# LMCache/LMCache

Measured on NVIDIA H100. Metric: kv_encode_decode_raw_GBps, higher is better.
Workload: dtype f32->u8 (bf16 KV)

## Files before the change

### lmcache_b200/csrc/codec.cu

```cuda
#include <cuda_bf16.h>
#include <cuda_fp16.h>
#include <cuda_runtime.h>
#include <stdint.h>
#include <stdlib.h>
#include <string.h>

#include <algorithm>
#include <vector>

#include "ac_core.cuh"
#include "common.cuh"

namespace b200kv {

constexpr int CT = 128;
constexpr int SPW = 6;
constexpr int SYMW = 43;
constexpr int PAIRW = 33;
constexpr int TEMPW_FUSED = 40;
constexpr int TEMPW_SPLIT = 132;
constexpr int TEMPW_FUSED_RANS = 48;
constexpr int CODER_AC = 0, CODER_RANS = 1;
constexpr int CODER_RANS_COMPACT = 2;
constexpr int kHdrRowWords = 8;
// ... 6 lines not shown
    int32_t L, H, D, C, dtype;
    int32_t n_chunks, chunk_tokens, last_chunk_tokens, tpp;
    int32_t tiles_full, tempw;
    int32_t stage_bytes;
    int32_t coder;
    int32_t compact;
    int32_t ppl;
    uint8_t* out;
    int64_t out_stride;
    uint64_t* sizes_out;
    uint32_t* temp;
    uint32_t* rstate;
    uint32_t* tile_tot;
    unsigned long long* totals;
    unsigned int* err;
    int32_t lb, nlay;
    uint8_t* arena;
    int64_t arena_bytes;
    unsigned long long* chunk_base;
    unsigned long long* cursor;
    unsigned int* fail_from;
    unsigned long long* ptotal;
    int64_t* seg;
    int32_t layers_left;
};
static_assert(sizeof(EncParams) < kMaxParamBytes, "EncParams must stay under 4 KB of kernel parameters");

__device__ __forceinline__ int launch_plane(const EncParams& P, int local) {
    return local + (local < P.nlay ? P.lb : P.L - P.nlay + P.lb);
}
// ... 47 lines not shown
    if (nb > 16) m |= (uint32_t)*reinterpret_cast<const uint16_t*>(p + 2) << 16;
    if (nb <= 8) m &= 0xffu;
    return nb >= 32 ? m : m & ((1u << nb) - 1u);
}

__device__ __forceinline__ int chunk_tokens_of(const EncParams& P, int j) {
    return j == P.n_chunks - 1 ? P.last_chunk_tokens : P.chunk_tokens;
}

template <bool PAGED>
__device__ __forceinline__ int64_t tok_row(const int64_t* slot_map, int64_t tok) {
    if constexpr (PAGED) return __ldg(slot_map + tok);
    else return tok;
}

template <bool VEC, bool PAGED>
__global__ void __launch_bounds__(256) absmax_kernel(EncParams P, int64_t total_tokens) {
    const int64_t warp = (blockIdx.x * (int64_t)blockDim.x + threadIdx.x) >> 5;
    const int lane = threadIdx.x & 31;
    const int64_t nrows = (int64_t)P.ppl * P.nlay * total_tokens;
    if (warp >= nrows) return;
    const int nl = launch_plane(P, (int)(warp / total_tokens));
    const int64_t T = warp % total_tokens;
    const uint16_t* row = P.pt.p[nl] + tok_row<PAGED>(P.slot_map, P.tok_begin + T) * P.sT;
    uint32_t m = 0;
    if (VEC) {
        const int vec_per_head = P.D >> 3;
        const int nvec = P.H * vec_per_head;
        for (int v = lane; v < nvec; v += 32) {
            const int h = v / vec_per_head, dv = v - h * vec_per_head;
            const uint4 q = __ldg(reinterpret_cast<const uint4*>(row + (int64_t)h * P.sH + dv * 8));
            const uint32_t w[4] = {q.x, q.y, q.z, q.w};
#pragma unroll
            for (int k = 0; k < 4; ++k) {
                const uint32_t a = w[k] & 0x7fff7fffu;
                m = max(m, max(a & 0xffffu, a >> 16));
            }
        }
    } else {
        for (int c = lane; c < P.C; c += 32) {
            const int h = c / P.D, d = c - h * P.D;
            m = max(m, (uint32_t)(__ldg(row + (int64_t)h * P.sH + d) & 0x7fffu));
        }
    }
    m = __reduce_max_sync(0xffffffffu, m);
    if (lane == 0) {
        const int j = (int)(T / P.chunk_tokens);
        const int tj = chunk_tokens_of(P, j);
        const Layout lo = layout_of(P, tj);
        uint16_t* maxes = reinterpret_cast<uint16_t*>(P.out + (int64_t)j * P.out_stride + lo.off_maxes);
        maxes[(int64_t)nl * tj + (T - (int64_t)j * P.chunk_tokens)] = (uint16_t)m;
    }
}

__device__ __forceinline__ uint32_t block_excl_scan(uint32_t v, uint32_t* s_warp, uint32_t* total) {
    const int lane = threadIdx.x & 31, wid = threadIdx.x >> 5;
    uint32_t inc = v;
#pragma unroll
    for (int o = 1; o < 32; o <<= 1) {
        uint32_t n = __shfl_up_sync(0xffffffffu, inc, o);
// ... 82 lines not shown
        for (int k = BT - 1; k >= 0; --k)
            if (tk + k < gt) f(q[k]);
    };
    load(xa, nbatch - 1);
    for (int b = nbatch - 1; b >= 0; b -= 2) {
        if (b >= 1) load(xb, b - 1);
        use(xa, b);
        if (b >= 1) {
            if (b >= 2) load(xa, b - 2);
            use(xb, b - 1);
        }
    }
}


template <bool FUSED, int DT, bool PAGED, int CODER>
__global__ void __launch_bounds__(CT, FUSED ? 7 : 4) encode_kernel(EncParams P) {
    extern __shared__ __align__(128) uint32_t smem[];
    constexpr int ROWS_W = FUSED ? CT * SYMW : 0;
    constexpr int TAB_W = FUSED ? (CT * kLp * 2 + 3) / 4 : CT * PAIRW;
    uint32_t* rows = smem;
    uint32_t* tab = smem + ROWS_W;
    float* fac = reinterpret_cast<float*>(smem + ((ROWS_W + TAB_W + 3) & ~3));
    __shared__ uint32_t s_warp[CT / 32];

    const int tid = threadIdx.x;
    TileId id;
    if (!decode_tile(P, blockIdx.x, &id)) return;
    const int NL = P.ppl * P.L;
    const int j = id.j, nl = id.nl, ct = id.ct, t = id.t, gt = id.gt;
    const int c = ct * CT + tid;
    const bool active = c < P.C;
    const int ncols = min(CT, P.C - ct * CT);

    uint8_t* cont = P.out + (int64_t)j * P.out_stride;
    const Layout lo = layout_of(P, t);
    const uint16_t* maxes = reinterpret_cast<const uint16_t*>(cont + lo.off_maxes) + (int64_t)nl * t + id.tok0;
    const float maxq = P.pt.maxq[nl];
    const int64_t s1 = P.sT;
    for (int i = tid; i < gt; i += CT)
        fac[i] = FUSED ? quant_factor_safe(maxq, half_to_float(maxes[i], DT)) : quant_factor(maxq, half_to_float(maxes[i], DT));
    if (FUSED) for (int i = gt + tid; i < kGroup + 8; i += CT) fac[i] = 0.0f;

    const int h = active ? c / P.D : 0;
    const int64_t tokabs = P.tok_begin + (int64_t)j * P.chunk_tokens + id.tok0;
    const uint16_t* cbase = P.pt.p[nl] + (int64_t)h * P.sH + (active ? c - h * P.D : 0);
    const uint16_t* src = cbase + (PAGED ? 0 : tokabs * P.sT);
    uint32_t* trow = P.temp + ((int64_t)blockIdx.x * CT + tid) * P.tempw;
    uint32_t cap = (uint32_t)P.tempw;
    asm volatile("" : "+l"(trow), "+r"(cap));
    uint32_t len = 0u, hlen = 0u;

    if (FUSED) {
        uint32_t* myrow = rows + tid * SYMW;
        uint16_t* cdfr = reinterpret_cast<uint16_t*>(tab);
        uint16_t* crow = cdfr + tid * kLp;
        uint16_t* hist = crow;
#pragma unroll
        for (int i = 0; i < kLp; ++i) crow[i] = 0;
        if (!PAGED) {
            const int lines_per_tok = (ncols * 2 + 127) >> 7;
            const uint16_t* tile0 = P.pt.p[nl] + (P.tok_begin + (int64_t)j * P.chunk_tokens + id.tok0) * P.sT +
                                    (int64_t)((ct * CT) / P.D) * P.sH + ((ct * CT) % P.D);
// ... 76 lines not shown
            uint32_t mask = 0u;
#pragma unroll
            for (int i = 0; i < 32; ++i) mask |= (cnt[i] != 0u ? 1u : 0u) << i;
            const uint32_t wany = __reduce_or_sync(__activemask(), mask);
            CdfAccum2 acc;
            acc.init();
#pragma unroll
            for (uint32_t i = 0; i < 32u; ++i) {
                crow[i] = (uint16_t)acc.value(i);
                if ((wany >> i) & 1u) acc.absorb(fac[cnt[i]]);
            }
            crow[32] = (uint16_t)acc.value(32u);
            if (P.compact) {
                uint32_t w0, w1;
                hlen = build_stream_header(cnt, mask, wany, 2 * ((int)maxq + 1), trow, w0, w1);
                reinterpret_cast<uint2*>(P.rstate)[((int64_t)blockIdx.x * CT + tid) * 2] = make_uint2(w0, w1);
            }
        }
        __syncthreads();
        if (!P.compact) {
            uint16_t* dstc = reinterpret_cast<uint16_t*>(cont + lo.off_cdf) + ((int64_t)nl * P.C + ct * CT) * kLp;
            for (int e = tid; e < ncols * kLp; e += CT) dstc[e] = cdfr[e];
        }
        if (active && CODER == CODER_RANS) {
            uint32_t x = kRansLow;
            const uint16_t* const wend = reinterpret_cast<const uint16_t*>(trow) + 2 * P.tempw;
            int32_t nk = 0;
            const char* const cb = reinterpret_cast<const char*>(crow);
            auto code = [&](uint32_t word, int k) {
                const uint32_t o = (k == 0 ? word << 1 : word >> (5 * k - 1)) & 62u;
                const uint32_t c_lo = *reinterpret_cast<const uint16_t*>(cb + o);
                const uint32_t c_hi = *reinterpret_cast<const uint16_t*>(cb + o + 2);
                rans_put(x, nk, wend, c_lo, c_hi - c_lo);
            };
            int w = (gt - 1) / SPW;
            {
                const uint32_t word = myrow[w];
                for (int k = gt - 1 - w * SPW; k >= 0; --k) code(word, k);
            }
            for (--w; w >= 0; --w) {
                const uint32_t word = myrow[w];
#pragma unroll
                for (int k = SPW - 1; k >= 0; --k) code(word, k);
            }
            if (P.compact) reinterpret_cast<uint2*>(P.rstate)[((int64_t)blockIdx.x * CT + tid) * 2 + 1] = make_uint2(x, hlen);
            else P.rstate[(int64_t)blockIdx.x * CT + tid] = x;
            len = hlen + 4u - 2u * (uint32_t)nk;
        } else if (active) {
            EncState2 st;
            st.init();
            int tk = 0;
            for (int w = 0; tk < gt; ++w) {
                const uint32_t word = myrow[w];
                if (tk + SPW <= gt) {
#pragma unroll
                    for (int k = 0; k < SPW; ++k) {
                        const uint32_t sidx = (word >> (5 * k)) & 31u;
                        const uint32_t c_lo = crow[sidx];
                        enc_symbol2(st, c_lo, (uint32_t)crow[sidx + 1u] - c_lo, trow, cap);
                    }
                    tk += SPW;
// ... 19 lines not shown
#pragma unroll
            for (int i = 0; i < kLp; ++i) cv[i] = prow[i] & 0xffffu;
#pragma unroll
            for (int i = 0; i < 32; ++i) {
                const uint32_t hi = (i == 31) ? 0x10000u : cv[i + 1];
                prow[i] = cv[i] | ((hi - cv[i]) << 16);
            }
            if (CODER == CODER_RANS) {
                uint32_t x = kRansLow;
                const uint16_t* const wend = reinterpret_cast<const uint16_t*>(trow) + 2 * TEMPW_SPLIT;
                int32_t nk = 0;
                for_each_symbol_rev<DT, PAGED, 4>(cbase, P.slot_map, tokabs, s1, gt, fac, maxq, [&](uint32_t q) {
                    const uint32_t pr = prow[q];
                    rans_put(x, nk, wend, pr & 0xffffu, pr >> 16);
                });
                P.rstate[(int64_t)blockIdx.x * CT + tid] = x;
                len = 4u - 2u * (uint32_t)nk;
            } else {
                EncState2 st;
                st.init();
                for_each_symbol<DT, PAGED, 4>(cbase, P.slot_map, tokabs, s1, gt, fac, maxq, [&](uint32_t q) {
                    const uint32_t pr = prow[q];
                    enc_symbol2(st, pr & 0xffffu, pr >> 16, trow, cap);
                });
                len = enc_finish2(st, trow, cap);
                if (st.w > cap) atomicOr(&P.err[j], 1u);
            }
        }
    }

    if (active) store_len(cont + lo.off_lengths, ((int64_t)id.g * NL + nl) * P.C + c, len, P.compact != 0);
    uint32_t tile_total;
    (void)block_excl_scan(len, s_warp, &tile_total);
    if (tid == 0) P.tile_tot[(int64_t)j * P.tiles_full + id.tile_in_chunk] = tile_total;
}

template <int DT, bool PAGED>
__global__ void __launch_bounds__(CT) cdf_kernel(EncParams P) {
    extern __shared__ __align__(128) uint32_t smem[];
    uint32_t* cnts = smem;
    float* fac = reinterpret_cast<float*>(cnts + CT * PAIRW);
    const int tid = threadIdx.x;
    const int NL = P.ppl * P.L;
    const uint32_t per_chunk = (uint32_t)NL * P.tpp;
    const uint32_t j = blockIdx.x / per_chunk;
    const uint32_t rem = blockIdx.x - j * per_chunk;
    const int nl = (int)(rem / P.tpp);
    const int ct = (int)(rem - (uint32_t)nl * P.tpp);
    const int t = chunk_tokens_of(P, (int)j);
// ... 855 lines not shown
        }
        cudaEventRecord(g_prof_ev[slot][0], stream);
    }
    ~ProfScope() {
        if (!g_prof_on) return;
        cudaEventRecord(g_prof_ev[slot][1], stream);
        g_prof_have[slot] = true;
    }
};

static int enc_tempw(bool fused, int coder, bool compact = false) {
    if (compact) return TEMPW_FUSED_RANS_HDR;
    return fused ? (coder == CODER_RANS ? TEMPW_FUSED_RANS : TEMPW_FUSED) : TEMPW_SPLIT;
}

static size_t enc_ws_layout(int64_t n_tiles_alloc, int n_chunks, int tempw, int coder, bool compact, size_t* off_tot,
                            size_t* off_totals, size_t* off_err, size_t* off_state, size_t* off_temp) {
    size_t o = 0;
    *off_tot = o;    o += (size_t)n_tiles_alloc * 4;  o = (o + 255) & ~(size_t)255;
    *off_totals = o; o += (size_t)n_chunks * 8;       o = (o + 255) & ~(size_t)255;
    *off_err = o;    o += (size_t)n_chunks * 4;       o = (o + 255) & ~(size_t)255;
    *off_state = o;  o += coder == CODER_RANS ? (size_t)n_tiles_alloc * CT * (compact ? 16 : 4) : 0;  o = (o + 255) & ~(size_t)255;
    *off_temp = o;   o += (size_t)n_tiles_alloc * CT * (size_t)tempw * 4;
    return (o + 255) & ~(size_t)255;
}

struct EnclWs { size_t err, ptotal, cbase, state, tot, totals, rstate, temp, bytes; };
static EnclWs encl_ws_layout(int n_chunks, int64_t call_tiles) {
    EnclWs w;
    size_t o = 0;
    auto take = [&](size_t* off, size_t n) { *off = o; o = (o + n + 255) & ~(size_t)255; };
    take(&w.err, (size_t)n_chunks * 4);
    take(&w.ptotal, (size_t)n_chunks * 8);
    take(&w.cbase, (size_t)n_chunks * 8);
    take(&w.state, 16);
    take(&w.tot, (size_t)call_tiles * 4);
    take(&w.totals, (size_t)n_chunks * 8);
    take(&w.rstate, (size_t)call_tiles * CT * 16);
    take(&w.temp, (size_t)call_tiles * CT * TEMPW_FUSED_RANS_HDR * 4);
    w.bytes = o;
    return w;
}

constexpr uint32_t kEncPlanMagic = 0x4e4c5045u;
struct LayerSet {
    static constexpr int kWords = B200KV_MAX_PLANES / 2 / 64;
    uint64_t w[kWords];
    static LayerSet range(int a, int b) {
        LayerSet s;
        for (int i = 0; i < kWords; ++i) {
            const int lo = std::max(a - 64 * i, 0), hi = std::min(b - 64 * i, 64);
            s.w[i] = lo >= hi ? 0ull : (hi - lo == 64 ? ~0ull : ((1ull << (hi - lo)) - 1ull) << lo);
// ... 19 lines not shown
        return n;
    }
};
static_assert(LayerSet::kWords * 64 == B200KV_MAX_PLANES / 2, "one bit per layer");
struct EncPlan {
    uint32_t magic;
    int32_t max_layers;
    LayerSet done;
    EncParams P;
};
static_assert(sizeof(EncPlan) <= sizeof(b200kv_encode_plan_t), "b200kv_encode_plan_t too small");

constexpr size_t kSmemFused = (size_t)(((CT * SYMW + (CT * kLp * 2 + 3) / 4 + 3) & ~3) + kGroup + 8) * 4;
constexpr int kStageRans = 12 * 1024;

static int launch_absmax(const EncParams& P, const b200kv_kv_desc* kv, int64_t total_tokens, cudaStream_t stream) {
    bool vec = (kv->D % 8 == 0) && (kv->sT % 8 == 0) && (kv->sH % 8 == 0);
    for (int nl = 0; nl < P.ppl * P.L && vec; ++nl) vec = (reinterpret_cast<uintptr_t>(P.pt.p[nl]) & 15) == 0;
    const bool paged = P.slot_map != nullptr;
    const int64_t rows = (int64_t)P.ppl * P.nlay * total_tokens;
    const int64_t blocks = (rows + 7) / 8;
    B2_REQUIRE(blocks < (1ll << 31), "too many rows in one call");
    if (vec && !paged) absmax_kernel<true, false><<<(unsigned)blocks, 256, 0, stream>>>(P, total_tokens);
    else if (vec) absmax_kernel<true, true><<<(unsigned)blocks, 256, 0, stream>>>(P, total_tokens);
    else if (!paged) absmax_kernel<false, false><<<(unsigned)blocks, 256, 0, stream>>>(P, total_tokens);
    else absmax_kernel<false, true><<<(unsigned)blocks, 256, 0, stream>>>(P, total_tokens);
    B2_CHECK_CUDA(cudaGetLastError());
    return 0;
}

static size_t dec_ws_layout(int64_t tiles_max, int n_chunks, int NP, size_t* off_tb, size_t* off_pt) {
    size_t o = ((size_t)n_chunks * sizeof(DecChunk) + 255) & ~(size_t)255;
    *off_tb = o;
    o += (size_t)n_chunks * (size_t)tiles_max * 8;
    o = (o + 255) & ~(size_t)255;
    *off_pt = o;
    if (NP > kInlinePlanes) o = (o + sizeof(PlaneTable) + 255) & ~(size_t)255;
    return o;
}

constexpr uint32_t kPlanMagic = 0x4e4c5044u;
// ... 70 lines not shown
    return 0;
}

int64_t b200kv_encode_workspace_bytes(int32_t L, int32_t H, int32_t D, int32_t chunk_tokens, int32_t n_chunks,
                                      int32_t coder) {
    if (L <= 0 || H <= 0 || D <= 0 || chunk_tokens <= 0 || n_chunks <= 0) return -2;
    const int ppl = (coder & B200KV_KV_LATENT) ? 1 : 2;
    coder &= 0xff;
    const bool compact = coder == CODER_RANS_COMPACT;
    if (compact) coder = CODER_RANS;
    if (coder != CODER_AC && coder != CODER_RANS) return -2;
    if (compact && chunk_tokens > kGroup) return -2;
    if (ppl == 1 && !compact) return -2;
    const int64_t G = (chunk_tokens + kGroup - 1) / kGroup;
    const int64_t n_tiles = (int64_t)n_chunks * G * ppl * L * tiles_per_plane(H * D);
    size_t a, b, c, d, e;
    return (int64_t)enc_ws_layout(n_tiles, n_chunks, enc_tempw(chunk_tokens <= kGroup, coder, compact), coder, compact, &a, &b, &c, &d, &e);
}

int64_t b200kv_decode_workspace_bytes(int32_t L, int32_t H, int32_t D, int32_t chunk_tokens, int32_t n_chunks) {
    if (L <= 0 || H <= 0 || D <= 0 || chunk_tokens <= 0 || n_chunks <= 0) return -2;
    const int64_t G = (chunk_tokens + kGroup - 1) / kGroup;
    const int64_t tiles_max = G * 2 * L * tiles_per_plane(H * D);
    size_t a, b;
    return (int64_t)dec_ws_layout(tiles_max, n_chunks, 2 * L, &a, &b);
}

int b200kv_encode_chunks(const b200kv_kv_desc* kv, int64_t tok_begin, int32_t n_chunks, int32_t chunk_tokens,
                         int32_t last_chunk_tokens, const float* key_bins, const float* value_bins, int32_t coder,
                         void* out, int64_t out_stride, uint64_t* sizes_out, void* workspace, int64_t workspace_bytes,
                         void* stream_) {
    cudaStream_t stream = static_cast<cudaStream_t>(stream_);
// ... 24 lines not shown
    P.out_stride = out_stride;
    P.sizes_out = sizes_out;
    P.lb = 0; P.nlay = P.L;
    P.arena = nullptr; P.arena_bytes = 0; P.chunk_base = nullptr; P.cursor = nullptr; P.fail_from = nullptr;
    P.ptotal = nullptr; P.seg = nullptr; P.layers_left = 0;
    const Layout lo = make_layout(P.L, P.C, chunk_tokens, P.compact, P.ppl);
    B2_REQUIRE(out_stride >= lo.off_payload + 16, "out_stride smaller than the fixed container sections");

    const int64_t G = lo.ngroups;
    const int64_t per_group = (int64_t)P.ppl * P.L * P.tpp;
    const int64_t tiles_full = G * per_group;
    const int64_t n_tiles = (int64_t)n_chunks * tiles_full;
    const bool fused = chunk_tokens <= kGroup;
    P.tiles_full = (int32_t)tiles_full;
    P.tempw = enc_tempw(fused, coder, P.compact != 0);
    size_t off_tot, off_totals, off_err, off_state, off_temp;
    const size_t need = enc_ws_layout(n_tiles, n_chunks, P.tempw, coder, P.compact != 0, &off_tot, &off_totals, &off_err, &off_state,
                                      &off_temp);
    B2_REQUIRE(workspace != nullptr && workspace_bytes >= (int64_t)need, "workspace too small");
    B2_REQUIRE(n_tiles < (1ll << 31) && tiles_full < (1ll << 31), "too many tiles in one call");
    uint8_t* ws = static_cast<uint8_t*>(workspace);
    P.tile_tot = reinterpret_cast<uint32_t*>(ws + off_tot);
    P.totals = reinterpret_cast<unsigned long long*>(ws + off_totals);
    P.err = reinterpret_cast<unsigned int*>(ws + off_err);
    P.temp = reinterpret_cast<uint32_t*>(ws + off_temp);
    P.rstate = reinterpret_cast<uint32_t*>(ws + off_state);
    B2_CHECK_CUDA(cudaMemsetAsync(ws, 0, off_state, stream));

    const int64_t total_tokens = (int64_t)(n_chunks - 1) * chunk_tokens + last_chunk_tokens;
    for (int i = 0; i <= kProfFinalize; ++i) g_prof_have[i] = false;
    {
        ProfScope prof(kProfAbsmax, stream);
        if (int rc = launch_absmax(P, kv, total_tokens, stream)) return rc;
    }
    const size_t smem_fused = kSmemFused;
    const size_t smem_split = (size_t)(((CT * PAIRW + 3) & ~3) + kGroup + 4) * 4;
    const size_t smem_cdf = (size_t)(CT * PAIRW + kGroup) * 4;
#define B2_LAUNCH_ENC1(FUSED, DT, PAGED, CODER, SMEM)                                                      \
    do {                                                                                                   \
        B2_CHECK_CUDA(cudaFuncSetAttribute(encode_kernel<FUSED, DT, PAGED, CODER>,                         \
                                           cudaFuncAttributeMaxDynamicSharedMemorySize, (int)(SMEM)));     \
        encode_kernel<FUSED, DT, PAGED, CODER><<<(unsigned)n_tiles, CT, (SMEM), stream>>>(P);              \
    } while (0)
#define B2_LAUNCH_ENC(FUSED, DT, PAGED, SMEM)                                                              \
    do {                                                                                                   \
        if (coder == CODER_RANS) B2_LAUNCH_ENC1(FUSED, DT, PAGED, CODER_RANS, SMEM);                       \
        else B2_LAUNCH_ENC1(FUSED, DT, PAGED, CODER_AC, SMEM);                                             \
    } while (0)
#define B2_LAUNCH_ENC2(FUSED, SMEM)                                                                        \
    do {                                                                                                   \
        if (P.dtype == B200KV_DT_BF16) { if (paged) B2_LAUNCH_ENC(FUSED, 0, true, SMEM); else B2_LAUNCH_ENC(FUSED, 0, false, SMEM); } \
        else { if (paged) B2_LAUNCH_ENC(FUSED, 1, true, SMEM); else B2_LAUNCH_ENC(FUSED, 1, false, SMEM); } \
    } while (0)
    if (fused) {
        ProfScope prof(kProfEncode, stream);
        B2_LAUNCH_ENC2(true, smem_fused);
    } else {
        const unsigned cdf_blocks = (unsigned)((int64_t)n_chunks * per_group);
        {
            ProfScope prof(kProfCdf, stream);
            if (P.dtype == B200KV_DT_BF16) {
                if (paged) cdf_kernel<0, true><<<cdf_blocks, CT, smem_cdf, stream>>>(P);
                else cdf_kernel<0, false><<<cdf_blocks, CT, smem_cdf, stream>>>(P);
            } else {
                if (paged) cdf_kernel<1, true><<<cdf_blocks, CT, smem_cdf, stream>>>(P);
                else cdf_kernel<1, false><<<cdf_blocks, CT, smem_cdf, stream>>>(P);
            }
        }
        B2_CHECK_CUDA(cudaGetLastError());
        ProfScope prof(kProfEncode, stream);
        B2_LAUNCH_ENC2(false, smem_split);
// ... 8 lines not shown
        if (coder == CODER_RANS && !hint_mid) P.stage_bytes = 12 * 1024;
        B2_CHECK_CUDA(cudaFuncSetAttribute(compact_kernel, cudaFuncAttributeMaxDynamicSharedMemorySize, P.stage_bytes));
        enc_scan_kernel<<<(unsigned)n_chunks, 1024, 0, stream>>>(P);
        compact_kernel<<<(unsigned)n_tiles, CT, (size_t)P.stage_bytes, stream>>>(P);
        finalize_kernel<<<(n_chunks + 127) / 128, 128, 0, stream>>>(P);
    }
    B2_CHECK_CUDA(cudaGetLastError());
    return 0;
}

int64_t b200kv_encode_layers_workspace_bytes(int32_t L, int32_t H, int32_t D, int32_t chunk_tokens, int32_t n_chunks,
                                             int32_t max_layers) {
    if (L <= 0 || H <= 0 || D <= 0 || chunk_tokens <= 0 || chunk_tokens > kGroup || n_chunks <= 0 || max_layers <= 0 ||
        max_layers > L)
        return -2;
    return (int64_t)encl_ws_layout(n_chunks, (int64_t)n_chunks * 2 * max_layers * tiles_per_plane(H * D)).bytes;
}

int b200kv_encode_layers_plan(const b200kv_kv_desc* kv, int64_t tok_begin, int32_t n_chunks, int32_t chunk_tokens,
                              int32_t last_chunk_tokens, const float* key_bins, const float* value_bins, int32_t coder,
                              void* arena, int64_t arena_bytes, void* fixed_out, int64_t fixed_stride, int64_t* seg_sizes_out,
                              uint64_t* sizes_out, int32_t max_layers, void* workspace, int64_t workspace_bytes,
                              b200kv_encode_plan_t* plan_out, void* stream_) {
    cudaStream_t stream = static_cast<cudaStream_t>(stream_);
    B2_REQUIRE(plan_out != nullptr, "plan is NULL");
    EncPlan* plan = reinterpret_cast<EncPlan*>(plan_out);
    plan->magic = 0u;
    EncParams& P = plan->P;
    B2_REQUIRE(key_bins && value_bins, "bins are NULL");
    B2_REQUIRE((coder & 0xff) == CODER_RANS_COMPACT,
               "the layer-wise encode writes compact containers only (B200KV_CODER_RANS_COMPACT)");
// ... 14 lines not shown
    P.tpp = tiles_per_plane(P.C);
    P.coder = CODER_RANS;
    P.compact = 1;
    P.tempw = TEMPW_FUSED_RANS_HDR;
    P.stage_bytes = kStageRans;
    const Layout lo = make_layout(P.L, P.C, chunk_tokens, 1, P.ppl);
    B2_REQUIRE(fixed_stride >= lo.off_payload, "fixed_stride smaller than the fixed container sections");
    P.out = static_cast<uint8_t*>(fixed_out);
    P.out_stride = fixed_stride;
    P.sizes_out = sizes_out;
    P.arena = static_cast<uint8_t*>(arena);
    P.arena_bytes = arena_bytes;
    P.seg = seg_sizes_out;
    const int64_t call_tiles = (int64_t)n_chunks * P.ppl * max_layers * P.tpp;
    B2_REQUIRE(call_tiles < (1ll << 31), "too many tiles in one call");
    const EnclWs w = encl_ws_layout(n_chunks, call_tiles);
    B2_REQUIRE(workspace != nullptr && workspace_bytes >= (int64_t)w.bytes, "workspace too small");
    uint8_t* ws = static_cast<uint8_t*>(workspace);
    P.err = reinterpret_cast<unsigned int*>(ws + w.err);
    P.ptotal = reinterpret_cast<unsigned long long*>(ws + w.ptotal);
    P.chunk_base = reinterpret_cast<unsigned long long*>(ws + w.cbase);
    P.cursor = reinterpret_cast<unsigned long long*>(ws + w.state);
    P.fail_from = reinterpret_cast<unsigned int*>(ws + w.state + 8);
    P.tile_tot = reinterpret_cast<uint32_t*>(ws + w.tot);
    P.totals = reinterpret_cast<unsigned long long*>(ws + w.totals);
    P.rstate = reinterpret_cast<uint32_t*>(ws + w.rstate);
    P.temp = reinterpret_cast<uint32_t*>(ws + w.temp);
    B2_CHECK_CUDA(cudaMemsetAsync(ws, 0, w.tot, stream));
    B2_CHECK_CUDA(cudaMemsetAsync(fixed_out, 0, (size_t)fixed_stride * n_chunks, stream));
    encl_init_kernel<<<1, 1, 0, stream>>>(P);
    B2_CHECK_CUDA(cudaGetLastError());
    B2_CHECK_CUDA(cudaFuncSetAttribute(compact_kernel, cudaFuncAttributeMaxDynamicSharedMemorySize, P.stage_bytes));
    plan->max_layers = max_layers;
    plan->done = LayerSet::range(0, 0);
    plan->magic = kEncPlanMagic;
    return 0;
}

int b200kv_encode_layers(b200kv_encode_plan_t* plan_in, int32_t layer_begin, int32_t layer_end, void* stream_) {
    cudaStream_t stream = static_cast<cudaStream_t>(stream_);
    B2_REQUIRE(plan_in != nullptr, "plan is NULL");
    EncPlan* plan = reinterpret_cast<EncPlan*>(plan_in);
    B2_REQUIRE(plan->magic == kEncPlanMagic, "not a plan made by b200kv_encode_layers_plan");
    EncParams P = plan->P;
    B2_REQUIRE(layer_begin >= 0 && layer_begin < layer_end && layer_end <= P.L, "layer range out of range");
    B2_REQUIRE(layer_end - layer_begin <= plan->max_layers, "more layers than the plan's workspace holds");
    const LayerSet bits = LayerSet::range(layer_begin, layer_end);
    B2_REQUIRE(!plan->done.intersects(bits), "a layer of the range was encoded before");
    P.lb = layer_begin;
    P.nlay = layer_end - layer_begin;
    P.layers_left = P.L - plan->done.count() - bits.count();
    P.tiles_full = P.ppl * P.nlay * P.tpp;
    const int64_t n_tiles = (int64_t)P.n_chunks * P.tiles_full;
    const int64_t total_tokens = (int64_t)(P.n_chunks - 1) * P.chunk_tokens + P.last_chunk_tokens;
    b200kv_kv_desc kv{};
    kv.D = P.D; kv.sT = P.sT; kv.sH = P.sH;
    if (int rc = launch_absmax(P, &kv, total_tokens, stream)) return rc;
#define B2_LAUNCH_ENCL(DT, PAGED)                                                                                      \
    do {                                                                                                               \
        B2_CHECK_CUDA(cudaFuncSetAttribute(encode_kernel<true, DT, PAGED, CODER_RANS>,                                 \
                                           cudaFuncAttributeMaxDynamicSharedMemorySize, (int)kSmemFused));             \
        encode_kernel<true, DT, PAGED, CODER_RANS><<<(unsigned)n_tiles, CT, kSmemFused, stream>>>(P);                  \
    } while (0)
    if (P.dtype == B200KV_DT_BF16) { if (P.slot_map) B2_LAUNCH_ENCL(0, true); else B2_LAUNCH_ENCL(0, false); }
    else { if (P.slot_map) B2_LAUNCH_ENCL(1, true); else B2_LAUNCH_ENCL(1, false); }
#undef B2_LAUNCH_ENCL
    B2_CHECK_CUDA(cudaGetLastError());
    enc_scan_kernel<<<(unsigned)P.n_chunks, 1024, 0, stream>>>(P);
    place_kernel<<<1, 1024, 0, stream>>>(P);
    compact_kernel<<<(unsigned)n_tiles, CT, (size_t)P.stage_bytes, stream>>>(P);
    B2_CHECK_CUDA(cudaGetLastError());
    plan->done.add(bits);
    return 0;
}

int b200kv_encode_layers_finish(const b200kv_encode_plan_t* plan_in, void* stream_) {
    cudaStream_t stream = static_cast<cudaStream_t>(stream_);
    B2_REQUIRE(plan_in != nullptr, "plan is NULL");
    const EncPlan* plan = reinterpret_cast<const EncPlan*>(plan_in);
    B2_REQUIRE(plan->magic == kEncPlanMagic, "not a plan made by b200kv_encode_layers_plan");
    EncParams P = plan->P;
    B2_REQUIRE(plan->done == LayerSet::range(0, P.L), "a layer was never encoded");
// ... 251 lines not shown
```

Measured before the change: 424.9.

## Fuse absmax into persistent encode kernel with ticket scheduler and ready flags

Replaces the separate absmax launch in the fused encode path with a persistent encode kernel. Its blocks pull work tickets that interleave absmax row-groups and encode tiles, with a lead of a few units so absmax runs ahead. Encode tiles spin on per-unit release/acquire ready counters before reading maxes. This removes a kernel boundary and lets the absmax reads overlap with encoding. It adds atomic ticket contention, spin-waits and a deadlock risk if scheduling assumptions fail. The absmax row loop is also batched four loads deep.

```diff
diff --git a/fused_absmax_bench.py b/fused_absmax_bench.py
--- /dev/null
+++ b/fused_absmax_bench.py
@@ -0,0 +1,109 @@
+#!/usr/bin/env python
+import argparse
+import ctypes
+import json
+import os
+import subprocess
+import sys
+
+ROOT = os.path.dirname(os.path.abspath(__file__))
+sys.path.insert(0, ROOT)
+
+MODEL = "lmsys/longchat-7b-16k"
+L, D = 32, 128
+
+
+def card():
+    try:
+        q = subprocess.run(["nvidia-smi", "--query-gpu=name,power.limit,clocks.max.sm", "--format=csv,noheader"],
+                           capture_output=True, text=True, timeout=30).stdout.strip().splitlines()
+        return q[0] if q else None
+    except (OSError, subprocess.SubprocessError):
+        return None
+
+
+def main():
+    ap = argparse.ArgumentParser()
+    ap.add_argument("--tokens", type=int, default=8192)
+    ap.add_argument("--chunk", type=int, default=256)
+    ap.add_argument("--heads", type=int, default=32)
+    ap.add_argument("--wave", type=int, default=8)
+    ap.add_argument("--steps", type=int, default=10)
+    ap.add_argument("--warmup", type=int, default=3)
+    ap.add_argument("--data", default="kv8d")
+    args = ap.parse_args()
+
+    import torch
+
+    import __graft_entry__ as ge
+    ge.build_cuda()
+    import bench
+    bench.H, bench.C = args.heads, args.heads * D
+    from lmcache_b200 import _native as N
+    from lmcache_b200.codec import CacheGenCodec, KvView
+
+    dev = torch.device("cuda", 0)
+    torch.cuda.set_device(dev)
+    H = args.heads
+    T, cs = args.tokens, args.chunk
+    n_chunks = (T + cs - 1) // cs
+    W = max(1, min(args.wave, n_chunks))
+    lib = N.lib()
+    codec = CacheGenCodec(MODEL)
+    kv = bench.synth_kv_torch(T, dev, 1236, args.data)
+    view = KvView.from_blob(kv, "vllm")
+    stride = codec.out_stride(L, H, D, cs)
+    staging = torch.empty(stride * W + N.READ_SLACK, dtype=torch.uint8, device=dev)
+    stream = torch.cuda.current_stream()
+    waves = [(c0, min(W * cs, T - c0 * cs)) for c0 in range(0, n_chunks, W)]
+
+    def step():
+        for c0, nt in waves:
+            codec.encode_async(view, c0 * cs, nt, cs, out=staging)
+
+    for _ in range(args.warmup):
+        step()
+    torch.cuda.synchronize()
+
+    ev0, ev1 = torch.cuda.Event(enable_timing=True), torch.cuda.Event(enable_timing=True)
+    call_ms = []
+    for _ in range(args.steps):
+        ev0.record(stream)
+        step()
+        ev1.record(stream)
+        torch.cuda.synchronize()
+        call_ms.append(ev0.elapsed_time(ev1))
+
+    lib.b200kv_profile_enable(1)
+    slots = {k: [] for k in N.PROFILE_SLOTS}
+    for _ in range(args.steps):
+        tot = {}
+        for c0, nt in waves:
+            codec.encode_async(view, c0 * cs, nt, cs, out=staging)
+            buf = (ctypes.c_float * 8)()
+            N.check(lib.b200kv_profile_last(buf, 8))
+            for i, name in enumerate(N.PROFILE_SLOTS):
+                if buf[i] >= 0:
+                    tot[name] = tot.get(name, 0.0) + buf[i]
+        for k, v in tot.items():
+            slots[k].append(v)
+    lib.b200kv_profile_enable(0)
+    torch.cuda.synchronize()
+
+    def med(v):
+        v = sorted(v)
+        return v[len(v) // 2]
+
+    s = {k: round(med(v), 4) for k, v in slots.items() if v}
+    raw = L * 2 * T * H * D * 2
+    line = {"card": card(), "shape": f"{L}L/{H}H/{D}D {T} tokens, chunk {cs}, waves of {W}", "data": args.data,
+            "steps": args.steps, "encode_call_ms": round(med(call_ms), 4),
+            "encode_call_ms_min_max": [round(min(call_ms), 4), round(max(call_ms), 4)],
+            "encode_call_GBps": round(raw / (med(call_ms) * 1e-3) / 1e9, 1), "slots_ms": s,
+            "absmax_plus_encode_ms": round(s.get("absmax", 0.0) + s.get("encode", 0.0), 4),
+            "encode_only_ms": s.get("encode")}
+    print(json.dumps(line))
+
+
+if __name__ == "__main__":
+    main()
diff --git a/lmcache_b200/csrc/codec.cu b/lmcache_b200/csrc/codec.cu
--- a/lmcache_b200/csrc/codec.cu
+++ b/lmcache_b200/csrc/codec.cu
@@ -44,6 +44,9 @@
     uint32_t* tile_tot;
     unsigned long long* totals;
     unsigned int* err;
+    unsigned int* ticket;
+    unsigned int* ready;
+    int32_t vec;
     int32_t lb, nlay;
     uint8_t* arena;
     int64_t arena_bytes;
@@ -121,6 +124,40 @@
     else return tok;
 }
 
+template <bool VEC>
+__device__ __forceinline__ uint32_t row_absmax(const EncParams& P, const uint16_t* row, int lane) {
+    uint32_t m = 0;
+    if (VEC) {
+        const int vec_per_head = P.D >> 3;
+        const int nvec = P.H * vec_per_head;
+        constexpr int B = 4;
+        for (int v0 = lane; v0 < nvec; v0 += 32 * B) {
+            uint4 q[B];
+#pragma unroll
+            for (int b = 0; b < B; ++b) {
+                const int v = v0 + 32 * b;
+                const int h = v / vec_per_head, dv = v - h * vec_per_head;
+                q[b] = v < nvec ? __ldg(reinterpret_cast<const uint4*>(row + (int64_t)h * P.sH + dv * 8)) : make_uint4(0, 0, 0, 0);
+            }
+#pragma unroll
+            for (int b = 0; b < B; ++b) {
+                const uint32_t w[4] = {q[b].x, q[b].y, q[b].z, q[b].w};
+#pragma unroll
+                for (int k = 0; k < 4; ++k) {
+                    const uint32_t a = w[k] & 0x7fff7fffu;
+                    m = max(m, max(a & 0xffffu, a >> 16));
+                }
+            }
+        }
+    } else {
+        for (int c = lane; c < P.C; c += 32) {
+            const int h = c / P.D, d = c - h * P.D;
+            m = max(m, (uint32_t)(__ldg(row + (int64_t)h * P.sH + d) & 0x7fffu));
+        }
+    }
+    return __reduce_max_sync(0xffffffffu, m);
+}
+
 template <bool VEC, bool PAGED>
 __global__ void __launch_bounds__(256) absmax_kernel(EncParams P, int64_t total_tokens) {
     const int64_t warp = (blockIdx.x * (int64_t)blockDim.x + threadIdx.x) >> 5;
@@ -130,27 +167,7 @@
     const int nl = launch_plane(P, (int)(warp / total_tokens));
     const int64_t T = warp % total_tokens;
     const uint16_t* row = P.pt.p[nl] + tok_row<PAGED>(P.slot_map, P.tok_begin + T) * P.sT;
-    uint32_t m = 0;
-    if (VEC) {
-        const int vec_per_head = P.D >> 3;
-        const int nvec = P.H * vec_per_head;
-        for (int v = lane; v < nvec; v += 32) {
-            const int h = v / vec_per_head, dv = v - h * vec_per_head;
-            const uint4 q = __ldg(reinterpret_cast<const uint4*>(row + (int64_t)h * P.sH + dv * 8));
-            const uint32_t w[4] = {q.x, q.y, q.z, q.w};
-#pragma unroll
-            for (int k = 0; k < 4; ++k) {
-                const uint32_t a = w[k] & 0x7fff7fffu;
-                m = max(m, max(a & 0xffffu, a >> 16));
-            }
-        }
-    } else {
-        for (int c = lane; c < P.C; c += 32) {
-            const int h = c / P.D, d = c - h * P.D;
-            m = max(m, (uint32_t)(__ldg(row + (int64_t)h * P.sH + d) & 0x7fffu));
-        }
-    }
-    m = __reduce_max_sync(0xffffffffu, m);
+    const uint32_t m = row_absmax<VEC>(P, row, lane);
     if (lane == 0) {
         const int j = (int)(T / P.chunk_tokens);
         const int tj = chunk_tokens_of(P, j);
@@ -263,19 +280,45 @@
 }
 
 
-template <bool FUSED, int DT, bool PAGED, int CODER>
-__global__ void __launch_bounds__(CT, FUSED ? 7 : 4) encode_kernel(EncParams P) {
-    extern __shared__ __align__(128) uint32_t smem[];
+constexpr int kAbsRows = 8;
+constexpr int kAbsItems = kGroup / kAbsRows;
+constexpr int kAbsLead = 8;
+
+template <bool PAGED>
+__device__ __forceinline__ void absmax_item(const EncParams& P, int unit, int item) {
+    const int nloc = P.ppl * P.nlay;
+    const int j = unit / nloc;
+    const int nl = launch_plane(P, unit - j * nloc);
+    const int tj = chunk_tokens_of(P, j);
+    const Layout lo = layout_of(P, tj);
+    uint16_t* maxes = reinterpret_cast<uint16_t*>(P.out + (int64_t)j * P.out_stride + lo.off_maxes) + (int64_t)nl * tj;
+    const int64_t tok0 = P.tok_begin + (int64_t)j * P.chunk_tokens;
+    const int lane = threadIdx.x & 31;
+    const int r0 = item * kAbsRows, r1 = min(tj, (item + 1) * kAbsRows);
+    for (int r = r0 + (threadIdx.x >> 5); r < r1; r += CT / 32) {
+        const uint16_t* row = P.pt.p[nl] + tok_row<PAGED>(P.slot_map, tok0 + r) * P.sT;
+        const uint32_t m = P.vec ? row_absmax<true>(P, row, lane) : row_absmax<false>(P, row, lane);
+        if (lane == 0) {
+            maxes[r] = (uint16_t)m;
+            __threadfence();
+        }
+    }
+    __syncthreads();
+    if (threadIdx.x == 0) asm volatile("red.release.gpu.global.add.u32 [%0], 1;" ::"l"(P.ready + unit) : "memory");
+}
+
+template <bool FUSED, int DT, bool PAGED, int CODER, class TileOf>
+__device__ __forceinline__ void encode_tile(const EncParams& P, TileOf tile_of, uint32_t* smem, uint32_t* s_warp) {
     constexpr int ROWS_W = FUSED ? CT * SYMW : 0;
     constexpr int TAB_W = FUSED ? (CT * kLp * 2 + 3) / 4 : CT * PAIRW;
     uint32_t* rows = smem;
     uint32_t* tab = smem + ROWS_W;
     float* fac = reinterpret_cast<float*>(smem + ((ROWS_W + TAB_W + 3) & ~3));
-    __shared__ uint32_t s_warp[CT / 32];
 
     const int tid = threadIdx.x;
     TileId id;
-    if (!decode_tile(P, blockIdx.x, &id)) return;
+    const uint32_t tile = tile_of();
+    if (!decode_tile(P, tile, &id)) return;
     const int NL = P.ppl * P.L;
     const int j = id.j, nl = id.nl, ct = id.ct, t = id.t, gt = id.gt;
     const int c = ct * CT + tid;
@@ -287,15 +330,30 @@
     const uint16_t* maxes = reinterpret_cast<const uint16_t*>(cont + lo.off_maxes) + (int64_t)nl * t + id.tok0;
     const float maxq = P.pt.maxq[nl];
     const int64_t s1 = P.sT;
+    if (FUSED) {
+        if (tid == 0) {
+            const unsigned int* rd = P.ready + tile / (uint32_t)P.tpp;
+            uint32_t ns = 32u;
+            for (;;) {
+                uint32_t v;
+                asm volatile("ld.acquire.gpu.global.u32 %0, [%1];" : "=r"(v) : "l"(rd) : "memory");
+                if (v >= (uint32_t)kAbsItems) break;
+                __nanosleep(ns);
+                ns = min(2u * ns, 1024u);
+            }
+        }
+        __syncthreads();
+    }
     for (int i = tid; i < gt; i += CT)
-        fac[i] = FUSED ? quant_factor_safe(maxq, half_to_float(maxes[i], DT)) : quant_factor(maxq, half_to_float(maxes[i], DT));
+        fac[i] = FUSED ? quant_factor_safe(maxq, half_to_float(__ldcg(maxes + i), DT))
+                       : quant_factor(maxq, half_to_float(maxes[i], DT));
     if (FUSED) for (int i = gt + tid; i < kGroup + 8; i += CT) fac[i] = 0.0f;
 
     const int h = active ? c / P.D : 0;
     const int64_t tokabs = P.tok_begin + (int64_t)j * P.chunk_tokens + id.tok0;
     const uint16_t* cbase = P.pt.p[nl] + (int64_t)h * P.sH + (active ? c - h * P.D : 0);
     const uint16_t* src = cbase + (PAGED ? 0 : tokabs * P.sT);
-    uint32_t* trow = P.temp + ((int64_t)blockIdx.x * CT + tid) * P.tempw;
+    uint32_t* trow = P.temp + ((int64_t)tile * CT + tid) * P.tempw;
     uint32_t cap = (uint32_t)P.tempw;
     asm volatile("" : "+l"(trow), "+r"(cap));
     uint32_t len = 0u, hlen = 0u;
@@ -402,7 +460,7 @@
             if (P.compact) {
                 uint32_t w0, w1;
                 hlen = build_stream_header(cnt, mask, wany, 2 * ((int)maxq + 1), trow, w0, w1);
-                reinterpret_cast<uint2*>(P.rstate)[((int64_t)blockIdx.x * CT + tid) * 2] = make_uint2(w0, w1);
+                reinterpret_cast<uint2*>(P.rstate)[((int64_t)tile_of() * CT + tid) * 2] = make_uint2(w0, w1);
             }
         }
         __syncthreads();
@@ -431,8 +489,8 @@
 #pragma unroll
                 for (int k = SPW - 1; k >= 0; --k) code(word, k);
             }
-            if (P.compact) reinterpret_cast<uint2*>(P.rstate)[((int64_t)blockIdx.x * CT + tid) * 2 + 1] = make_uint2(x, hlen);
-            else P.rstate[(int64_t)blockIdx.x * CT + tid] = x;
+            if (P.compact) reinterpret_cast<uint2*>(P.rstate)[((int64_t)tile_of() * CT + tid) * 2 + 1] = make_uint2(x, hlen);
+            else P.rstate[(int64_t)tile_of() * CT + tid] = x;
             len = hlen + 4u - 2u * (uint32_t)nk;
         } else if (active) {
             EncState2 st;
@@ -482,7 +540,7 @@
                     const uint32_t pr = prow[q];
                     rans_put(x, nk, wend, pr & 0xffffu, pr >> 16);
                 });
-                P.rstate[(int64_t)blockIdx.x * CT + tid] = x;
+                P.rstate[(int64_t)tile_of() * CT + tid] = x;
                 len = 4u - 2u * (uint32_t)nk;
             } else {
                 EncState2 st;
@@ -501,6 +559,42 @@
     uint32_t tile_total;
     (void)block_excl_scan(len, s_warp, &tile_total);
     if (tid == 0) P.tile_tot[(int64_t)j * P.tiles_full + id.tile_in_chunk] = tile_total;
+}
+
+template <bool FUSED, int DT, bool PAGED, int CODER>
+__global__ void __launch_bounds__(CT, FUSED ? 7 : 4) encode_kernel(EncParams P) {
+    extern __shared__ __align__(128) uint32_t smem[];
+    __shared__ uint32_t s_warp[CT / 32];
+    if constexpr (!FUSED) {
+        encode_tile<false, DT, PAGED, CODER>(P, [] { return (uint32_t)blockIdx.x; }, smem, s_warp);
+    } else {
+        constexpr uint32_t kWorkDone = 0xffffffffu, kWorkNone = 0xfffffffeu, kWorkAbsmax = 0x80000000u;
+        __shared__ uint32_t s_work;
+        for (;;) {
+            __syncthreads();
+            if (threadIdx.x == 0) {
+                const uint32_t units = (uint32_t)P.n_chunks * (uint32_t)(P.ppl * P.nlay);
+                const uint32_t step = (uint32_t)(kAbsItems + P.tpp);
+                const uint32_t k = atomicAdd(P.ticket, 1u);
+                const uint32_t s = k / step, r = k - s * step;
+                uint32_t w = kWorkNone;
+                if (s >= units + kAbsLead) w = kWorkDone;
+                else if (r < (uint32_t)kAbsItems) { if (s < units) w = kWorkAbsmax | (s * kAbsItems + r); }
+                else if (s >= (uint32_t)kAbsLead) w = (s - kAbsLead) * (uint32_t)P.tpp + (r - kAbsItems);
+                s_work = w;
+            }
+            __syncthreads();
+            const uint32_t w = s_work;
+            if (w == kWorkDone) break;
+            if (w == kWorkNone) continue;
+            if (w & kWorkAbsmax) {
+                const uint32_t a = w & ~kWorkAbsmax;
+                absmax_item<PAGED>(P, (int)(a / kAbsItems), (int)(a % kAbsItems));
+            } else {
+                encode_tile<true, DT, PAGED, CODER>(P, [] { return *static_cast<volatile uint32_t*>(&s_work); }, smem, s_warp);
+            }
+        }
+    }
 }
 
 template <int DT, bool PAGED>
@@ -1386,19 +1480,21 @@
     return fused ? (coder == CODER_RANS ? TEMPW_FUSED_RANS : TEMPW_FUSED) : TEMPW_SPLIT;
 }
 
-static size_t enc_ws_layout(int64_t n_tiles_alloc, int n_chunks, int tempw, int coder, bool compact, size_t* off_tot,
-                            size_t* off_totals, size_t* off_err, size_t* off_state, size_t* off_temp) {
+static size_t enc_ws_layout(int64_t n_tiles_alloc, int n_chunks, int64_t n_units, int tempw, int coder, bool compact,
+                            size_t* off_tot, size_t* off_totals, size_t* off_err, size_t* off_sync, size_t* off_state,
+                            size_t* off_temp) {
     size_t o = 0;
     *off_tot = o;    o += (size_t)n_tiles_alloc * 4;  o = (o + 255) & ~(size_t)255;
     *off_totals = o; o += (size_t)n_chunks * 8;       o = (o + 255) & ~(size_t)255;
     *off_err = o;    o += (size_t)n_chunks * 4;       o = (o + 255) & ~(size_t)255;
+    *off_sync = o;   o += (size_t)(1 + n_units) * 4;  o = (o + 255) & ~(size_t)255;
     *off_state = o;  o += coder == CODER_RANS ? (size_t)n_tiles_alloc * CT * (compact ? 16 : 4) : 0;  o = (o + 255) & ~(size_t)255;
     *off_temp = o;   o += (size_t)n_tiles_alloc * CT * (size_t)tempw * 4;
     return (o + 255) & ~(size_t)255;
 }
 
-struct EnclWs { size_t err, ptotal, cbase, state, tot, totals, rstate, temp, bytes; };
-static EnclWs encl_ws_layout(int n_chunks, int64_t call_tiles) {
+struct EnclWs { size_t err, ptotal, cbase, state, tot, totals, sync, rstate, temp, bytes; };
+static EnclWs encl_ws_layout(int n_chunks, int64_t call_tiles, int64_t call_units) {
     EnclWs w;
     size_t o = 0;
     auto take = [&](size_t* off, size_t n) { *off = o; o = (o + n + 255) & ~(size_t)255; };
@@ -1408,6 +1504,7 @@
     take(&w.state, 16);
     take(&w.tot, (size_t)call_tiles * 4);
     take(&w.totals, (size_t)n_chunks * 8);
+    take(&w.sync, (size_t)(1 + call_units) * 4);
     take(&w.rstate, (size_t)call_tiles * CT * 16);
     take(&w.temp, (size_t)call_tiles * CT * TEMPW_FUSED_RANS_HDR * 4);
     w.bytes = o;
@@ -1457,9 +1554,14 @@
 constexpr size_t kSmemFused = (size_t)(((CT * SYMW + (CT * kLp * 2 + 3) / 4 + 3) & ~3) + kGroup + 8) * 4;
 constexpr int kStageRans = 12 * 1024;
 
-static int launch_absmax(const EncParams& P, const b200kv_kv_desc* kv, int64_t total_tokens, cudaStream_t stream) {
-    bool vec = (kv->D % 8 == 0) && (kv->sT % 8 == 0) && (kv->sH % 8 == 0);
+static bool rows_vec(const EncParams& P) {
+    bool vec = (P.D % 8 == 0) && (P.sT % 8 == 0) && (P.sH % 8 == 0);
     for (int nl = 0; nl < P.ppl * P.L && vec; ++nl) vec = (reinterpret_cast<uintptr_t>(P.pt.p[nl]) & 15) == 0;
+    return vec;
+}
+
+static int launch_absmax(const EncParams& P, int64_t total_tokens, cudaStream_t stream) {
+    const bool vec = P.vec != 0;
     const bool paged = P.slot_map != nullptr;
     const int64_t rows = (int64_t)P.ppl * P.nlay * total_tokens;
     const int64_t blocks = (rows + 7) / 8;
@@ -1468,6 +1570,28 @@
     else if (vec) absmax_kernel<true, true><<<(unsigned)blocks, 256, 0, stream>>>(P, total_tokens);
     else if (!paged) absmax_kernel<false, false><<<(unsigned)blocks, 256, 0, stream>>>(P, total_tokens);
     else absmax_kernel<false, true><<<(unsigned)blocks, 256, 0, stream>>>(P, total_tokens);
+    B2_CHECK_CUDA(cudaGetLastError());
+    return 0;
+}
+
+template <int DT, bool PAGED, int CODER>
+static int launch_encode_fused(const EncParams& P, cudaStream_t stream) {
+    static int occ = 0;
+    auto kern = encode_kernel<true, DT, PAGED, CODER>;
+    B2_CHECK_CUDA(cudaFuncSetAttribute(kern, cudaFuncAttributeMaxDynamicSharedMemorySize, (int)kSmemFused));
+    if (occ == 0) {
+        int n = 0;
+        B2_CHECK_CUDA(cudaOccupancyMaxActiveBlocksPerMultiprocessor(&n, kern, CT, kSmemFused));
+        B2_REQUIRE(n > 0, "encode_kernel does not fit on this device");
+        occ = n;
+    }
+    int dev = 0, sms = 0;
+    B2_CHECK_CUDA(cudaGetDevice(&dev));
+    B2_CHECK_CUDA(cudaDeviceGetAttribute(&sms, cudaDevAttrMultiProcessorCount, dev));
+    const int64_t tickets = ((int64_t)P.n_chunks * P.ppl * P.nlay + kAbsLead) * (kAbsItems + P.tpp);
+    B2_REQUIRE(tickets < (1ll << 31) - 2, "too many work items in one call");
+    const int64_t grid = std::min<int64_t>((int64_t)occ * sms, tickets);
+    kern<<<(unsigned)grid, CT, kSmemFused, stream>>>(P);
     B2_CHECK_CUDA(cudaGetLastError());
     return 0;
 }
@@ -1568,8 +1692,9 @@
     if (ppl == 1 && !compact) return -2;
     const int64_t G = (chunk_tokens + kGroup - 1) / kGroup;
     const int64_t n_tiles = (int64_t)n_chunks * G * ppl * L * tiles_per_plane(H * D);
-    size_t a, b, c, d, e;
-    return (int64_t)enc_ws_layout(n_tiles, n_chunks, enc_tempw(chunk_tokens <= kGroup, coder, compact), coder, compact, &a, &b, &c, &d, &e);
+    size_t a, b, c, d, e, f;
+    return (int64_t)enc_ws_layout(n_tiles, n_chunks, (int64_t)n_chunks * ppl * L, enc_tempw(chunk_tokens <= kGroup, coder, compact),
+                                  coder, compact, &a, &b, &c, &d, &e, &f);
 }
 
 int64_t b200kv_decode_workspace_bytes(int32_t L, int32_t H, int32_t D, int32_t chunk_tokens, int32_t n_chunks) {
@@ -1624,9 +1749,9 @@
     const bool fused = chunk_tokens <= kGroup;
     P.tiles_full = (int32_t)tiles_full;
     P.tempw = enc_tempw(fused, coder, P.compact != 0);
-    size_t off_tot, off_totals, off_err, off_state, off_temp;
-    const size_t need = enc_ws_layout(n_tiles, n_chunks, P.tempw, coder, P.compact != 0, &off_tot, &off_totals, &off_err, &off_state,
-                                      &off_temp);
+    size_t off_tot, off_totals, off_err, off_sync, off_state, off_temp;
+    const size_t need = enc_ws_layout(n_tiles, n_chunks, (int64_t)n_chunks * P.ppl * P.L, P.tempw, coder, P.compact != 0, &off_tot,
+                                      &off_totals, &off_err, &off_sync, &off_state, &off_temp);
     B2_REQUIRE(workspace != nullptr && workspace_bytes >= (int64_t)need, "workspace too small");
     B2_REQUIRE(n_tiles < (1ll << 31) && tiles_full < (1ll << 31), "too many tiles in one call");
     uint8_t* ws = static_cast<uint8_t*>(workspace);
@@ -1635,15 +1760,17 @@
     P.err = reinterpret_cast<unsigned int*>(ws + off_err);
     P.temp = reinterpret_cast<uint32_t*>(ws + off_temp);
     P.rstate = reinterpret_cast<uint32_t*>(ws + off_state);
+    P.ticket = reinterpret_cast<unsigned int*>(ws + off_sync);
+    P.ready = P.ticket + 1;
+    P.vec = rows_vec(P) ? 1 : 0;
     B2_CHECK_CUDA(cudaMemsetAsync(ws, 0, off_state, stream));
 
     const int64_t total_tokens = (int64_t)(n_chunks - 1) * chunk_tokens + last_chunk_tokens;
     for (int i = 0; i <= kProfFinalize; ++i) g_prof_have[i] = false;
-    {
+    if (!fused) {
         ProfScope prof(kProfAbsmax, stream);
-        if (int rc = launch_absmax(P, kv, total_tokens, stream)) return rc;
-    }
-    const size_t smem_fused = kSmemFused;
+        if (int rc = launch_absmax(P, total_tokens, stream)) return rc;
+    }
     const size_t smem_split = (size_t)(((CT * PAIRW + 3) & ~3) + kGroup + 4) * 4;
     const size_t smem_cdf = (size_t)(CT * PAIRW + kGroup) * 4;
 #define B2_LAUNCH_ENC1(FUSED, DT, PAGED, CODER, SMEM)                                                      \
@@ -1664,7 +1791,15 @@
     } while (0)
     if (fused) {
         ProfScope prof(kProfEncode, stream);
-        B2_LAUNCH_ENC2(true, smem_fused);
+        int rc;
+        if (P.dtype == B200KV_DT_BF16) {
+            if (paged) rc = coder == CODER_RANS ? launch_encode_fused<0, true, CODER_RANS>(P, stream) : launch_encode_fused<0, true, CODER_AC>(P, stream);
+            else rc = coder == CODER_RANS ? launch_encode_fused<0, false, CODER_RANS>(P, stream) : launch_encode_fused<0, false, CODER_AC>(P, stream);
+        } else {
+            if (paged) rc = coder == CODER_RANS ? launch_encode_fused<1, true, CODER_RANS>(P, stream) : launch_encode_fused<1, true, CODER_AC>(P, stream);
+            else rc = coder == CODER_RANS ? launch_encode_fused<1, false, CODER_RANS>(P, stream) : launch_encode_fused<1, false, CODER_AC>(P, stream);
+        }
+        if (rc) return rc;
     } else {
         const unsigned cdf_blocks = (unsigned)((int64_t)n_chunks * per_group);
         {
@@ -1703,7 +1838,8 @@
     if (L <= 0 || H <= 0 || D <= 0 || chunk_tokens <= 0 || chunk_tokens > kGroup || n_chunks <= 0 || max_layers <= 0 ||
         max_layers > L)
         return -2;
-    return (int64_t)encl_ws_layout(n_chunks, (int64_t)n_chunks * 2 * max_layers * tiles_per_plane(H * D)).bytes;
+    return (int64_t)encl_ws_layout(n_chunks, (int64_t)n_chunks * 2 * max_layers * tiles_per_plane(H * D),
+                                   (int64_t)n_chunks * 2 * max_layers).bytes;
 }
 
 int b200kv_encode_layers_plan(const b200kv_kv_desc* kv, int64_t tok_begin, int32_t n_chunks, int32_t chunk_tokens,
@@ -1748,7 +1884,7 @@
     P.seg = seg_sizes_out;
     const int64_t call_tiles = (int64_t)n_chunks * P.ppl * max_layers * P.tpp;
     B2_REQUIRE(call_tiles < (1ll << 31), "too many tiles in one call");
-    const EnclWs w = encl_ws_layout(n_chunks, call_tiles);
+    const EnclWs w = encl_ws_layout(n_chunks, call_tiles, (int64_t)n_chunks * P.ppl * max_layers);
     B2_REQUIRE(workspace != nullptr && workspace_bytes >= (int64_t)w.bytes, "workspace too small");
     uint8_t* ws = static_cast<uint8_t*>(workspace);
     P.err = reinterpret_cast<unsigned int*>(ws + w.err);
@@ -1760,6 +1896,9 @@
     P.totals = reinterpret_cast<unsigned long long*>(ws + w.totals);
     P.rstate = reinterpret_cast<uint32_t*>(ws + w.rstate);
     P.temp = reinterpret_cast<uint32_t*>(ws + w.temp);
+    P.ticket = reinterpret_cast<unsigned int*>(ws + w.sync);
+    P.ready = P.ticket + 1;
+    P.vec = rows_vec(P) ? 1 : 0;
     B2_CHECK_CUDA(cudaMemsetAsync(ws, 0, w.tot, stream));
     B2_CHECK_CUDA(cudaMemsetAsync(fixed_out, 0, (size_t)fixed_stride * n_chunks, stream));
     encl_init_kernel<<<1, 1, 0, stream>>>(P);
@@ -1786,20 +1925,11 @@
     P.layers_left = P.L - plan->done.count() - bits.count();
     P.tiles_full = P.ppl * P.nlay * P.tpp;
     const int64_t n_tiles = (int64_t)P.n_chunks * P.tiles_full;
-    const int64_t total_tokens = (int64_t)(P.n_chunks - 1) * P.chunk_tokens + P.last_chunk_tokens;
-    b200kv_kv_desc kv{};
-    kv.D = P.D; kv.sT = P.sT; kv.sH = P.sH;
-    if (int rc = launch_absmax(P, &kv, total_tokens, stream)) return rc;
-#define B2_LAUNCH_ENCL(DT, PAGED)                                                                                      \
-    do {                                                                                                               \
-        B2_CHECK_CUDA(cudaFuncSetAttribute(encode_kernel<true, DT, PAGED, CODER_RANS>,                                 \
-                                           cudaFuncAttributeMaxDynamicSharedMemorySize, (int)kSmemFused));             \
-        encode_kernel<true, DT, PAGED, CODER_RANS><<<(unsigned)n_tiles, CT, kSmemFused, stream>>>(P);                  \
-    } while (0)
-    if (P.dtype == B200KV_DT_BF16) { if (P.slot_map) B2_LAUNCH_ENCL(0, true); else B2_LAUNCH_ENCL(0, false); }
-    else { if (P.slot_map) B2_LAUNCH_ENCL(1, true); else B2_LAUNCH_ENCL(1, false); }
-#undef B2_LAUNCH_ENCL
-    B2_CHECK_CUDA(cudaGetLastError());
+    B2_CHECK_CUDA(cudaMemsetAsync(P.ticket, 0, (size_t)(1 + (int64_t)P.n_chunks * P.ppl * P.nlay) * 4, stream));
+    int rc;
+    if (P.dtype == B200KV_DT_BF16) rc = P.slot_map ? launch_encode_fused<0, true, CODER_RANS>(P, stream) : launch_encode_fused<0, false, CODER_RANS>(P, stream);
+    else rc = P.slot_map ? launch_encode_fused<1, true, CODER_RANS>(P, stream) : launch_encode_fused<1, false, CODER_RANS>(P, stream);
+    if (rc) return rc;
     enc_scan_kernel<<<(unsigned)P.n_chunks, 1024, 0, stream>>>(P);
     place_kernel<<<1, 1024, 0, stream>>>(P);
     compact_kernel<<<(unsigned)n_tiles, CT, (size_t)P.stage_bytes, stream>>>(P);
```

Result: faster. 443.9, median of 6 (+4.5%).
